# imedslab/OAProgressionMMF

Measured on AMD Instinct MI355X. Metric: knees/sec full XR+MRI+clin fusion train step, higher is better.
Workload: dtype f32; 1 GPU; syn3: XR1MR3C1CnnTrf train step (fwd+FocalLoss+bwd+Adam), per-GPU batch 8, global batch 8, BASELINE config 4 on BASELINE's synthetic tensors: XR 1x310x310 + 3 x MRI 1x160x384x384 (slice-major) + 9 clinical; random-init weights; parallelism=dp1, activation_recompute=012,012,01

## Files before the change

oaprogressionmmf_amd/csrc/koaf_conv.hip:

```cpp
#include "koaf_common.h"

namespace {

inline int64_t rup32(int64_t v) { return (v + 31) / 32 * 32; }

inline void set_fimg(KoafGemm* g, const KoafWImg* w, int R, int64_t K) {
    g->fmt = 1;
    g->A.fscale = KOAF_ACT_SCALE;
    g->B.amax = w->amax;
    if (!w->f) return;
    g->B.kind = 2; g->B.gather = 0;
    g->B.planes = w->f; g->B.ld = rup32(K); g->B.plane_stride = (int64_t)R * g->B.ld;
}

inline void set_aplanes(KoafOperand* a, const uint16_t* planes, int64_t plane_elems) {
    a->kind = 2; a->planes = planes; a->plane_stride = plane_elems; a->zeros = planes + 2 * plane_elems;
    a->ptr = nullptr; a->ptr2 = nullptr; a->tf = 0; a->sc = a->sh = a->sc2 = nullptr;
}

inline void set_gather(KoafOperand* o, int gather, int H, int W, int C, int CS, int PH, int PW, int KH, int KW, int stride, int pad_h,
                       int pad_w) {
    o->gather = gather;
    o->H = H; o->W = W; o->C = C; o->CS = CS;
    o->PH = PH; o->PW = PW;
    o->KH = KH; o->KW = KW; o->stride = stride; o->pad = pad_h; o->pad_w = pad_w;
}

inline bool is_pointwise(int KH, int KW, int stride, int pad) { return KH == 1 && KW == 1 && stride == 1 && pad == 0; }

struct WgradPlan { int bm, bn, splitk; };
inline WgradPlan wgrad_plan(int M, int N, int64_t K, int ctap, int batch) {
    WgradPlan p;
    p.bn = (N >= 128 && (ctap % 4) == 0) ? 128 : 64;
    p.bm = (M >= 128) ? 128 : 64;
    int64_t tiles = cdiv64(M, p.bm) * cdiv64(N, p.bn) * batch;
    int64_t sk = 1024 / tiles;
    int64_t kmax = cdiv64(K, 512);
    if (sk > kmax) sk = kmax;
    if (sk < 1) sk = 1;
    if (sk > 4096) sk = 4096;
    if (sk > 8) {
        int64_t best = sk & ~7ll;
        double beff = 0.0;
        for (int64_t c = ((sk * 3 / 4) + 7) & ~7ll; c <= 2 * sk && c <= kmax && c <= 4096; c += 8) {
            const int64_t blocks = tiles * c;
            const double eff = (double)blocks / (double)(cdiv64(blocks, 512) * 512);
            if (eff > beff + 0.02) { beff = eff; best = c; }
        }
        sk = best;
    }
    p.splitk = (int)sk;
    return p;
}

__global__ void __launch_bounds__(256) slab_reduce_b_kernel(const float* __restrict__ slabs, int ns, int64_t n,
                                                            float* __restrict__ out) {
    const int64_t i = ((int64_t)blockIdx.x * 256 + threadIdx.x) * 4;
    if (i >= n) return;
    const float* sb = slabs + (int64_t)blockIdx.y * ns * n;
    v4f a = *(const v4f*)(sb + i);
    for (int s = 1; s < ns; ++s) a += *(const v4f*)(sb + (int64_t)s * n + i);
    *(v4f*)(out + (int64_t)blockIdx.y * n + i) = a;
}

__global__ void __launch_bounds__(256) gconv_expand_kernel(const float* __restrict__ w, float* __restrict__ wexp,
                                                           int C, int Cg, float* __restrict__ amax) {
    const int64_t total = (int64_t)C * 9 * 64;
    unsigned mb = 0u;
    for (int64_t i = (int64_t)blockIdx.x * 256 + threadIdx.x; i < total; i += (int64_t)gridDim.x * 256) {
        const int ci = (int)(i & 63);
        int64_t r = i >> 6;
        const int tap = (int)(r % 9);
        const int co = (int)(r / 9);
        const int col = co & 63;
        const int g0 = (col / Cg) * Cg;
        float v = 0.f;
        if (ci >= g0 && ci < g0 + Cg) v = w[((int64_t)co * 9 + tap) * Cg + (ci - g0)];
        wexp[i] = v;
        mb = max(mb, koaf_absbits(v));
    }
    if (amax != nullptr) block_amax_raise_bits(mb, amax);
}
__global__ void __launch_bounds__(256) gconv_compress_kernel(const float* __restrict__ dwexp, float* __restrict__ dw,
                                                             int C, int Cg) {
    const int64_t total = (int64_t)C * 9 * Cg;
    for (int64_t i = (int64_t)blockIdx.x * 256 + threadIdx.x; i < total; i += (int64_t)gridDim.x * 256) {
        const int cg = (int)(i % Cg);
        int64_t r = i / Cg;
        const int tap = (int)(r % 9);
        const int co = (int)(r / 9);
        const int g0 = ((co & 63) / Cg) * Cg;
        dw[i] = dwexp[((int64_t)co * 9 + tap) * 64 + g0 + cg];
    }
}

}

int koaf_fwd_s2(const KoafGemm& g, void* stream);
static inline bool fwd_s2_ok(const KoafGemm& g, int KH, int KW, int stride, int pad, bool x_planes, bool tail, bool emit) {
    const KoafOperand& A = g.A;
    if (stride != 2 || KH != KW || !((KH == 1 && pad == 0) || (KH == 3 && pad == 1))) return false;
    if (g.fmt != 1 || g.B.kind != 2 || !g.B.planes || !g.B.amax || g.act16 != 0 || x_planes || tail || emit) return false;
    if (A.kind != 0 || A.gather != 1 || A.amax || (A.C % 32) != 0 || A.CS != A.C || (g.N % 128) != 0 || (g.M % 256) != 0 || g.K < 32) return false;
    if (A.tf != 0 && (A.tf != 1 || A.C > 1024 || !aligned16(A.sc) || !aligned16(A.sh))) return false;
    if (!aligned16(A.ptr) || !aligned16(g.B.planes) || !aligned16(g.C)) return false;
    return (int64_t)(g.M / (A.PH * A.PW)) * A.H * A.W < (1ll << 31);
}

extern "C" int koaf_conv2d_fwd(const float* x, const float* w, float* y, int32_t N, int32_t H, int32_t W, int32_t Cin,
                               int32_t Cout, int32_t KH, int32_t KW, int32_t stride, int32_t pad, const float* in_sc,
                               const float* in_sh, float* stats, int32_t* stats_rows, const float* stats_shift,
                               const KoafWImg* wimg, const uint16_t* x_planes, const KoafTail* tail, const KoafEmit* emit,
                               int32_t act16, void* stream) {
    KOAF_REQUIRE((x || x_planes) && w && y && N > 0 && Cin % 32 == 0 && Cout % 4 == 0, "koaf_conv2d_fwd: bad args (Cin=%d Cout=%d)",
                 Cin, Cout);
    KOAF_REQUIRE(!tail || (tail->idt && x && in_sc && in_sh && !x_planes && is_pointwise(KH, KW, stride, pad) && wimg &&
                           wimg->amax && wimg->f && (tail->idt_sc == nullptr) == (tail->idt_sh == nullptr)),
                 "koaf_conv2d_fwd: the fused bottleneck tail serves 1x1 / stride-1 convolutions with weight plane images, from x / in_sc / in_sh");
    KOAF_REQUIRE((in_sc == nullptr) == (in_sh == nullptr), "koaf_conv2d_fwd: in_sc/in_sh come together");
    const int OH = conv_out(H, KH, stride, pad), OW = conv_out(W, KW, stride, pad);
    const int64_t M = (int64_t)N * OH * OW;
    KOAF_REQUIRE(M < (1ll << 31), "koaf_conv2d_fwd: too many output pixels");
    KoafGemm g;
    zero_gemm(&g);
    g.A.ptr = x;
    g.A.kind = 0;
    if (is_pointwise(KH, KW, stride, pad) && !x_planes) {
        g.A.gather = 0;
        g.A.ld = Cin;
    } else
        set_gather(&g.A, 1, H, W, Cin, Cin, OH, OW, KH, KW, stride, pad, pad);
    if (in_sc) { g.A.tf = 1; g.A.sc = in_sc; g.A.sh = in_sh; }
    if (tail) { g.A.tf = 3; g.A.ptr2 = tail->idt; g.A.side = tail->y_out; g.A.sc2 = tail->idt_sc; g.A.sh2 = tail->idt_sc ? tail->idt_sh : nullptr; }
    g.B.ptr = w;
    g.B.kind = 0;
    g.B.ld = (int64_t)KH * KW * Cin;
    g.M = (int)M; g.N = Cout; g.K = KH * KW * Cin;
    if (wimg && wimg->amax) set_fimg(&g, wimg, Cout, g.K);
    if (x_planes) {
        KOAF_REQUIRE(g.A.gather == 1 && g.B.kind == 2, "koaf_conv2d_fwd: x_planes serve the gathered kernels and need wimg->f");
        set_aplanes(&g.A, x_planes, (int64_t)N * H * W * Cin);
    }
    g.C = y; g.ldc = Cout;
    g.stats = stats;
    g.stats_shift = stats ? stats_shift : nullptr;
    g.act16 = act16 ? 1 : 0;
    if (emit) {
        KOAF_REQUIRE(emit->planes && emit->sc && emit->sh && (Cout % 8) == 0, "koaf_conv2d_fwd: emit needs planes / sc / sh and Cout %% 8 == 0");
        g.out_planes = emit->planes; g.out_sc = emit->sc; g.out_sh = emit->sh; g.out_ps = M * Cout;
    }
    if (fwd_s2_ok(g, KH, KW, stride, pad, x_planes != nullptr, tail != nullptr, emit != nullptr)) {
        if (stats_rows) *stats_rows = g.M / 128;
        return koaf_fwd_s2(g, stream);
    }
    if (stats_rows) *stats_rows = koaf_gemm_part_rows(&g);
    return koaf_gemm(&g, stream);
}

extern "C" int32_t koaf_conv2d_stats_rows(int64_t M, int32_t Cout) { return (int32_t)cdiv64(M, 64); }

static void set_apply(KoafOperand* a, const KoafBnApply* ap, int C) {
    a->ptr = ap->dz; a->ptr2 = ap->c; a->tf = 2;
    a->sc = ap->coef; a->sc2 = ap->coef + 2 * (int64_t)C; a->sh = ap->coef + 3 * (int64_t)C;
    a->amax = ap->amax;
}

static void set_bnb(KoafGemm* g, const KoafBnb* b, float* part) {
    if (!b) return;
    g->bnb_amax = b->dz_amax;
    g->bnb_mode = b->mode;
    g->bnb_c = b->c; g->bnb_y = b->y; g->bnb_sc = b->sc; g->bnb_sh = b->sh;
    g->bnb_mean = b->mean; g->bnb_invstd = b->invstd;
    g->bnb2_c = b->c2; g->bnb2_mean = b->mean2; g->bnb2_invstd = b->invstd2;
    g->bnb_part = part;
}

extern "C" int32_t koaf_conv2d_dgrad_bnb_rows(int32_t N, int32_t H, int32_t W, int32_t Cin, int32_t stride) {
    if (stride == 2) {
        int64_t r = 0;
        for (int py = 0; py < 2; ++py)
            for (int px = 0; px < 2; ++px) r += cdiv64((int64_t)N * ((H - py + 1) / 2) * ((W - px + 1) / 2), 64);
        return (int32_t)r;
    }
    return (int32_t)cdiv64((int64_t)N * H * W, 64);
}

int koaf_dgrad_s2(const KoafGemm& g, void* stream);
static inline bool dgrad_s2_ok(const KoafGemm& g, int KH, int KW, int pad, int H, int W, const KoafBnb* bnb, bool dy_planes) {
    const KoafOperand& A = g.A;
    const bool f11 = KH == 1 && KW == 1 && pad == 0, f33 = KH == 3 && KW == 3 && pad == 1;
    if (!(f11 || f33) || (H & 1) || (W & 1) || (g.M % 256) != 0 || g.K < 32) return false;
    if (g.fmt != 1 || g.B.kind != 2 || !g.B.planes || !g.B.amax || !A.amax || g.act16 != 0 || g.residual) return false;
    if ((A.C % 32) != 0 || (g.N % 128) != 0 || !aligned16(g.C) || !aligned16(g.B.planes)) return false;
    if (bnb && (bnb->mode != 2 || bnb->c2 || !aligned16(bnb->c) || !aligned16(bnb->sc) || !aligned16(bnb->sh) || !aligned16(bnb->mean) ||
                !aligned16(bnb->invstd) || !aligned16(g.bnb_part)))
        return false;
    if (f33) return dy_planes && A.kind == 2 && aligned16(A.planes) && aligned16(A.zeros) && !(A.plane_stride & 7);
    if (dy_planes || bnb || A.kind != 0 || !aligned16(A.ptr)) return false;
    return A.tf == 0 || (A.tf == 2 && aligned16(A.ptr2) && aligned16(A.sc) && aligned16(A.sh) && aligned16(A.sc2));
}

extern "C" int koaf_conv2d_dgrad_bnb(const float* dy, const float* w, float* dx, int32_t N, int32_t H, int32_t W,
                                     int32_t Cin, int32_t Cout, int32_t KH, int32_t KW, int32_t stride, int32_t pad,
                                     const float* residual, const KoafBnb* bnb, float* part, int32_t* part_rows,
                                     const KoafWImg* wimg, const float* dy_amax, const KoafBnApply* dy_apply,
                                     const uint16_t* dy_planes, int32_t act16, void* stream) {
    KOAF_REQUIRE(!dy_planes || (wimg && wimg->amax && wimg->d && (dy_amax || dy_apply) && KH * KW > 1),
                 "koaf_conv2d_dgrad: dy_planes need the weight's D plane image, dy_amax and a gathered (KH*KW > 1) kernel");
    KOAF_REQUIRE((dy || dy_apply || dy_planes) && w && dx && N > 0 && Cout % 32 == 0 && Cin % 4 == 0, "koaf_conv2d_dgrad: bad args");
    KOAF_REQUIRE(!dy_apply || (dy_apply->dz && dy_apply->c && dy_apply->coef && dy_apply->amax && wimg && wimg->amax && wimg->d),
                 "koaf_conv2d_dgrad: dy_apply needs dz / c / coef / amax and the weight's D plane image");
    if (dy_apply) { dy = dy_apply->dz; dy_amax = dy_apply->amax; }
    if (bnb && bnb->dz_amax && hipMemsetAsync(bnb->dz_amax, 0, sizeof(float), (hipStream_t)stream) != hipSuccess) {
        koaf_set_error("koaf_conv2d_dgrad_bnb: memset failed");
        return KOAF_ELAUNCH;
    }
    const bool f16 = wimg && wimg->amax && dy_amax;
    const bool ps = f16 && wimg->d != nullptr;
    const uint16_t* w_dimg = ps ? wimg->d : nullptr;
    const int64_t dld = (int64_t)KH * KW * Cout, dps = (int64_t)Cin * dld;
    KOAF_REQUIRE(!bnb || (part && part_rows), "koaf_conv2d_dgrad_bnb: part / part_rows required");
    const int nsum = (bnb && bnb->c2) ? 3 : 2;
    int rows_done = 0;
    const int OH = conv_out(H, KH, stride, pad), OW = conv_out(W, KW, stride, pad);
    const int64_t M = (int64_t)N * H * W;
    KOAF_REQUIRE(M < (1ll << 31), "koaf_conv2d_dgrad: too many pixels");
    KoafGemm g;
    if (stride == 2) {
        bool all_done = false;
        for (int py = 0; py < 2 && !all_done; ++py)
            for (int px = 0; px < 2 && !all_done; ++px) {
                const int Hc = (H - py + 1) / 2, Wc = (W - px + 1) / 2;
                if (Hc <= 0 || Wc <= 0) continue;
                const int khs = (py + pad) & 1, kws = (px + pad) & 1;
                const int nkh = khs < KH ? (KH - khs + 1) / 2 : 0, nkw = kws < KW ? (KW - kws + 1) / 2 : 0;
                const int offy = (py + pad - khs) / 2, offx = (px + pad - kws) / 2;
                zero_gemm(&g);
                g.prec = 1;
                if (f16) { g.fmt = 1; g.A.amax = dy_amax; g.B.amax = wimg->amax; }
                g.A.ptr = dy; g.A.kind = 0;
                if (dy_apply) set_apply(&g.A, dy_apply, Cout);
                set_gather(&g.A, 2, OH, OW, Cout, Cout, Hc, Wc, nkh > 0 ? nkh : 1, nkw > 0 ? nkw : 1, 1, offy, offx);
                g.B.ptr = w + ((int64_t)khs * KW + kws) * Cin; g.B.kind = 1; g.B.gather = 3;
                g.B.C = Cout; g.B.ld = (int64_t)KH * KW * Cin;
                g.B.KW = g.A.KW; g.B.tap_stride = 2ll * Cin; g.B.tap_stride_h = 2ll * KW * Cin;
                if (ps) {
                    g.B.kind = 2; g.B.gather = 0;
                    g.B.planes = w_dimg + ((int64_t)khs * KW + kws) * Cout; g.B.ld = dld; g.B.plane_stride = dps;
                    g.B.tap_stride = 2ll * Cout; g.B.tap_stride_h = 2ll * KW * Cout;
                }
                if (dy_planes && nkh > 0 && nkw > 0) set_aplanes(&g.A, dy_planes, (int64_t)N * OH * OW * Cout);
                g.M = N * Hc * Wc; g.N = Cin; g.K = nkh * nkw * Cout;
                g.C = dx; g.ldc = Cin;
                g.residual = residual; g.ldr = Cin;
                g.cmap = 1; g.cm_PH = Hc; g.cm_PW = Wc; g.cm_H = H; g.cm_W = W; g.cm_py = py; g.cm_px = px;
                g.act16 = act16 ? 2 : 0;
                if (bnb) set_bnb(&g, bnb, part + (int64_t)rows_done * nsum * Cin);
                if (dgrad_s2_ok(g, KH, KW, pad, H, W, bnb, dy_planes != nullptr)) {
                    if (bnb) rows_done += g.M / 128;
                    int rc = koaf_dgrad_s2(g, stream);
                    if (rc != KOAF_OK) return rc;
                    all_done = KH == 1;
                    continue;
                }
                if (bnb) rows_done += koaf_gemm_part_rows(&g);
                int rc = koaf_gemm(&g, stream);
                if (rc != KOAF_OK) return rc;
            }
        if (part_rows) *part_rows = rows_done;
        return KOAF_OK;
    }
    zero_gemm(&g);
    g.prec = 1;
    if (f16) { g.fmt = 1; g.A.amax = dy_amax; g.B.amax = wimg->amax; }
    g.A.ptr = dy;
    g.A.kind = 0;
    if (dy_apply) set_apply(&g.A, dy_apply, Cout);
    g.B.ptr = w;
    g.B.kind = 1;
    if (is_pointwise(KH, KW, stride, pad)) {
        g.A.gather = 0;
        g.A.ld = Cout;
        g.B.gather = 0;
        g.B.ld = Cin;
    } else {
        set_gather(&g.A, 2, OH, OW, Cout, Cout, H, W, KH, KW, stride, pad, pad);
        g.B.gather = 3;
        g.B.C = Cout;
        g.B.ld = (int64_t)KH * KW * Cin;
        g.B.KW = KW;
        g.B.tap_stride = Cin;
        g.B.tap_stride_h = (int64_t)KW * Cin;
    }
    if (ps) {
        g.B.kind = 2; g.B.gather = 0; g.B.C = 0; g.B.tap_stride = g.B.tap_stride_h = 0;
        g.B.planes = w_dimg; g.B.ld = dld; g.B.plane_stride = dps;
    }
    if (dy_planes) set_aplanes(&g.A, dy_planes, (int64_t)N * OH * OW * Cout);
    g.M = (int)M; g.N = Cin; g.K = KH * KW * Cout;
    g.C = dx; g.ldc = Cin;
    g.residual = residual; g.ldr = Cin;
    if (bnb) {
        set_bnb(&g, bnb, part);
        *part_rows = koaf_gemm_part_rows(&g);
    }
    g.act16 = act16 ? 2 : 0;
// ... 204 lines not shown
```

oaprogressionmmf_amd/csrc/koaf_gemm.hip:

```cpp
#include "koaf_gemm_launch.h"
#include <stdlib.h>
#include <string.h>
#include <atomic>
#include <mutex>
#include <vector>

namespace {

__global__ void __launch_bounds__(256) slab_reduce_epi_kernel(const float* __restrict__ slabs, int nslab, int M, int N,
                                                              const float* __restrict__ bias,
                                                              const float* __restrict__ residual, int64_t ldr,
                                                              float* __restrict__ out, int64_t ldo) {
    const int N4 = N / 4;
    const int64_t total = (int64_t)M * N4;
    const int64_t n = (int64_t)M * N;
    for (int64_t i = (int64_t)blockIdx.x * 256 + threadIdx.x; i < total; i += (int64_t)gridDim.x * 256) {
        const int m = (int)(i / N4), c = (int)(i - (int64_t)m * N4) * 4;
        v4f a = *(const v4f*)(slabs + (int64_t)m * N + c);
        for (int s = 1; s < nslab; ++s) a += *(const v4f*)(slabs + (int64_t)s * n + (int64_t)m * N + c);
        if (bias) a += *(const v4f*)(bias + c);
        if (residual) a += *(const v4f*)(residual + (int64_t)m * ldr + c);
        *(v4f*)(out + (int64_t)m * ldo + c) = a;
    }
}

__global__ void __launch_bounds__(256) slab_reduce_kernel(const float* __restrict__ slabs, int nslab,
                                                          int64_t n, float* __restrict__ out) {
    __shared__ v4f red[4][64];
    const int cx = threadIdx.x & 63, gy = threadIdx.x >> 6;
    const int64_t i = ((int64_t)blockIdx.x * 64 + cx) * 4;
    const int s_per = (nslab + gridDim.y - 1) / gridDim.y;
    const int s0 = blockIdx.y * s_per, s1 = min(nslab, s0 + s_per);
    v4f a = {0.f, 0.f, 0.f, 0.f};
    if (i < n)
        for (int s = s0 + gy; s < s1; s += 4) a += *(const v4f*)(slabs + (int64_t)s * n + i);
    red[gy][cx] = a;
    __syncthreads();
    if (gy == 0 && i < n) {
        a = red[0][cx] + red[1][cx] + red[2][cx] + red[3][cx];
        if (gridDim.y == 1) *(v4f*)(out + i) = a;
        else *(v4f*)(out + (int64_t)blockIdx.y * n + i) = a;
    }
}

bool operand_vec_ok(const KoafOperand& o, int R, int K) {
    if (o.kind == 3) {
        return aligned16(o.planes) && aligned16(o.zeros) && o.zeros && !(o.plane_stride & 7) && !(o.bs0 & 7) && !(o.bs1 & 7) &&
               !(R & 7) && (o.gather ? (o.C > 0 && !(o.C & 7) && !(o.CS & 7) && o.KW > 0) : !(o.ld & 7));
    }
    if (o.kind == 2 && o.gather) {
        return aligned16(o.planes) && aligned16(o.zeros) && o.zeros && !(o.plane_stride & 7) && !(o.bs0 & 7) && !(o.bs1 & 7) &&
               o.C > 0 && !(o.C & 31) && !(o.CS & 7) && o.KW > 0 && (K % BK) == 0;
    }
    if (o.kind == 2) {
        if (!aligned16(o.planes) || (o.ld & 7) || (o.plane_stride & 7) || (o.bs0 & 7) || (o.bs1 & 7)) return false;
        if ((o.tap_stride & 7) || (o.tap_stride_h & 7) || o.C <= 0 || (o.C & 31) || o.KW <= 0) return false;
        return true;
    }
    if (!aligned16(o.ptr)) return false;
    if ((o.ld & 3) || (o.bs0 & 3) || (o.bs1 & 3)) return false;
    if (o.kind == 0) {
        if (K & 3) return false;
        if (o.gather && ((o.C & 31) || (o.CS & 3))) return false;
    } else {
        if (R & 3) return false;
        if (o.gather == 3 && ((o.C & 31) || (o.tap_stride & 3) || (o.tap_stride_h & 3))) return false;
        if (o.gather == 1 && ((o.C & 3) || (o.CS & 3))) return false;
    }
    if (o.tf && (!aligned16(o.sc) || !aligned16(o.sh))) return false;
    if (o.tf == 2 && (!aligned16(o.sc2) || !aligned16(o.ptr2))) return false;
    return true;
}

}

namespace {
std::atomic<int> g_log_on{0};
std::mutex g_log_mutex;
std::vector<KoafLaunchRec> g_log;
int64_t g_log_seen = 0;
constexpr size_t LOG_CAP = 4096;

}

void koaf_log_launch(const char* variant, const KoafGemm& g, dim3 grid, dim3 launched) {
    if (!g_log_on.load(std::memory_order_relaxed)) return;
    KoafLaunchRec r;
    memset(&r, 0, sizeof(r));
    strncpy(r.variant, variant, sizeof(r.variant) - 1);
    r.bm = g.bm; r.bn = g.bn;
    r.tiles = (int32_t)grid.x; r.grid_x = (int32_t)launched.x;
    r.splitk = (int32_t)launched.y; r.nbatch = (int32_t)launched.z;
    r.fmt = g.fmt; r.a_tf = g.A.tf; r.b_tf = g.B.tf; r.act16 = g.act16;
    r.M = g.M - g.m_base; r.N = g.N; r.K = g.K;
    r.emit = g.out_planes != nullptr;
    std::lock_guard<std::mutex> lock(g_log_mutex);
    ++g_log_seen;
    if (g_log.size() < LOG_CAP) g_log.push_back(r);
}

namespace {
int g_stream_mode = 1;
bool stream_ok(const KoafGemm& g) {
    return g_stream_mode == 1 && g.A.kind == 0 && g.A.gather == 0 && g.K >= 2 * BK && (g.K % (2 * BK)) == 0 && g.splitk == 1 &&
           g.nb0 * g.nb1 == 1 && (g.A.tf != 1 || g.K <= STREAM_TAB_K);
}
}

extern "C" int koaf_gemm_pick_tile(const KoafGemm* g, int32_t* bm, int32_t* bn) {
    int b_m = g->bm, b_n = g->bn;
    const int64_t batch = (int64_t)g->nb0 * g->nb1 * (g->splitk > 0 ? g->splitk : 1);
    if (b_n == 0) {
        b_n = (g->N >= 128) ? 128 : 64;
        if (g->B.kind == 1 && g->B.gather == 1 && (g->B.C % 64) != 0) b_n = 64;
    }
    if (b_m == 0) b_m = (g->M >= 128) ? 128 : 64;
    if (g->bm == 0 || g->bn == 0) {
        auto tiles = [&](int m, int n) { return cdiv64(g->M, m) * cdiv64(g->N, n) * batch; };
        constexpr int64_t fill = 384;
        if (g->bm == 0 && tiles(b_m, b_n) < fill && b_m == 128) b_m = 64;
        if (g->bn == 0 && tiles(b_m, b_n) < fill && b_n == 128) b_n = 64;
    }
    *bm = b_m;
    *bn = b_n;
    return KOAF_OK;
}

namespace {
int g_halo_mode = 1;

bool halo_ok(const KoafGemm& g) {
    const KoafOperand& a = g.A;
    return g_halo_mode != 0 && a.kind == 2 && (a.gather == 1 || a.gather == 2) && a.KH == 3 && a.KW == 3 && a.stride == 1 && a.pad == 1 &&
           a.pad_w == 1 && a.PH == a.H && a.PW == a.W && a.W <= halo_max_w(g.N >= 128 ? 128 : 64, 256) && a.H * a.W > 0 && (g.M % (a.H * a.W)) == 0 &&
           g.nb0 * g.nb1 == 1 && g.m_base == 0 && g.K == 9 * a.C && g.B.kind == 2 && g.fmt == 1 && !g.cmap && g.splitk == 1;
}

bool gemm_vec_ok(const KoafGemm& g) {
    bool vec = operand_vec_ok(g.A, g.M, g.K) && operand_vec_ok(g.B, g.N, g.K);
    if ((g.N & 3) || !aligned16(g.C) || (g.ldc & 3) || (g.cbs0 & 3) || (g.cbs1 & 3)) vec = false;
    if (g.residual && (!aligned16(g.residual) || (g.ldr & 3) || (g.rbs0 & 3) || (g.rbs1 & 3))) vec = false;
    if (g.bias && !aligned16(g.bias)) vec = false;
    return vec;
}

TilePlan plan_tiles(const KoafGemm& g) {
    TilePlan t;
    KoafGemm q = g;
    koaf_gemm_pick_tile(&q, &t.bm, &t.bn);
    t.vec = gemm_vec_ok(g);
    if (!t.vec) { t.bm = 64; t.bn = 64; }
    t.halo = t.vec && halo_ok(g);
    t.t2d = t.halo && g_halo_mode == 1 && g.A.C == 64 && (g.N == 64 || g.N == 128) && (g.A.W % 16) == 0 && (g.A.H % 8) == 0 &&
            g.A.zeros != nullptr;
    if (t.t2d) {
        t.halo = false;
        t.bm = 128;
        t.bn = 64;
    } else if (t.halo) {
        t.bn = g.N >= 128 ? 128 : 64;
        const bool fits128 = g.A.W <= halo_max_w(t.bn, 128);
        t.bm = (g_halo_mode == 3 || (g_halo_mode == 1 && g.A.C <= 64)) && fits128 ? 128 : 256;
    }
    t.part_rows = (int)cdiv64(g.M - g.m_base, t.bm);
    t.stream = t.vec && g.fmt == 1 && g.act16 == 0 && t.bm == 128 && operand_mode(g.A) == M_KC && operand_mode(g.B) == M_PS && !g.B.tf &&
               !(g.out_planes && g.A.tf == 2) && stream_ok(g);
    return t;
}
}

static void fill_defaults(KoafGemm& g) {
    if (g.nb0 < 1) g.nb0 = 1;
    if (g.nb1 < 1) g.nb1 = 1;
    if (g.splitk < 1) g.splitk = 1;
    if (g.A.CS == 0) g.A.CS = g.A.C;
    if (g.B.CS == 0) g.B.CS = g.B.C;
    if (g.stats_ld == 0) g.stats_ld = g.N;
    if (g.B.kind == 2 && g.B.C == 0) { g.B.C = ((g.K + BK - 1) / BK) * BK; g.B.KW = 1; }
}

namespace {
int launch_wplanes(const KoafGemm& g, const TilePlan& tp, dim3 grid, hipStream_t s) {
    switch (g.act16) {
        case 0: return koaf_launch_wplanes_act0(g, tp, grid, s);
        case 1: return koaf_launch_wplanes_act1(g, tp, grid, s);
        case 2: return koaf_launch_wplanes_act2(g, tp, grid, s);
    }
    return KOAF_NO_KERNEL;
}

int launch_planned(const KoafGemm& g, const TilePlan& tp, dim3 grid, hipStream_t s) {
    const int am = operand_mode(g.A), bm = operand_mode(g.B);
    if (g.out_planes && (tp.t2d || tp.halo)) { koaf_set_error("koaf_gemm: out_planes is not built for the 3x3 plane-image kernels"); return KOAF_EINVAL; }
    if ((tp.t2d || tp.halo) && g.act16 == 3) {
        koaf_set_error(tp.t2d ? "koaf_gemm: 2-D tile kernel with act16 = 3" : "koaf_gemm: halo kernel with act16 = 3");
        return KOAF_EINVAL;
    }
    if (tp.t2d || tp.halo) return launch_wplanes(g, tp, grid, s);
    if (g.fmt == 1) KOAF_REQUIRE(tp.vec, "koaf_gemm: the fp16 scheme needs the vector path (16-B aligned operands, K %% 4 == 0, N %% 4 == 0)");
    else if (!tp.vec && g.act16 != 0) { koaf_set_error("koaf_gemm: bf16 activation storage needs the vector path"); return KOAF_EINVAL; }
    int rc = KOAF_NO_KERNEL;
    if (tp.stream) rc = koaf_launch_stream(g, tp, grid, s);
    else if (g.out_planes) {
        if (g.fmt == 1 && am == M_KC && bm == M_PS) rc = launch_wplanes(g, tp, grid, s);
        if (rc == KOAF_NO_KERNEL) {
            koaf_set_error("koaf_gemm: out_planes is built for dense K-contiguous A x weight plane images on the fp16 scheme (1x1 forward convolutions); "
                           "got operand modes (%d,%d) tf=%d fmt=%d act16=%d", am, bm, g.A.tf, (int)(g.fmt == 1), g.act16);
            return KOAF_EINVAL;
        }
    }
    else if (bm == M_PS) rc = launch_wplanes(g, tp, grid, s);
    else if (am == M_PK) rc = koaf_launch_kmajor(g, tp, grid, s);
    else rc = g.fmt == 1 ? koaf_launch_fp16(g, tp, grid, s) : koaf_launch_bf16(g, tp, grid, s);
    if (rc == KOAF_NO_KERNEL) {
        koaf_set_error("koaf_gemm: operand mode pair (%d,%d) tf=(%d,%d) fmt=%d vec=%d act16=%d is not instantiated", am, bm, g.A.tf, g.B.tf,
                       (int)(g.fmt == 1), (int)tp.vec, g.act16);
        return KOAF_EINVAL;
    }
    return rc;
}
}

extern "C" int koaf_gemm_part_rows(const KoafGemm* gp) {
    KoafGemm g = *gp;
    fill_defaults(g);
    return plan_tiles(g).part_rows;
}

extern "C" int koaf_gemm(const KoafGemm* gp, void* stream) {
    KoafGemm g = *gp;
    KOAF_REQUIRE(g.M > 0 && g.N > 0 && g.K >= 0, "koaf_gemm: bad dims M=%d N=%d K=%d", g.M, g.N, g.K);
    KOAF_REQUIRE((g.A.kind >= 2 ? (const void*)g.A.planes : (const void*)g.A.ptr) &&
                 (g.B.kind >= 2 ? (const void*)g.B.planes : (const void*)g.B.ptr) && g.C, "koaf_gemm: null operand");
    fill_defaults(g);
    if (!g.status) g.status = koaf_status_ptr();
    KOAF_REQUIRE(!g.cmap || (g.splitk == 1 && !g.stats), "koaf_gemm: row map excludes split-K / stats");
    KOAF_REQUIRE(!g.bnb_mode || (g.splitk == 1 && !g.stats && g.nb0 * g.nb1 == 1 && g.bnb_c && g.bnb_mean &&
                                 g.bnb_invstd && g.bnb_part && (g.bnb_mode == 1 ? g.bnb_y != nullptr
                                                                                 : (g.bnb_sc && g.bnb_sh))),
                 "koaf_gemm: fused BN-backward epilogue needs c/mean/invstd/part (+y or sc/sh), no split-K/batch");
    KOAF_REQUIRE(g.splitk == 1 || (!g.bias && !g.residual && !g.stats),
                 "koaf_gemm: split-K writes raw slabs (no epilogue)");
    KOAF_REQUIRE((int64_t)g.nb0 * g.nb1 <= 65535 && g.splitk <= 65535, "koaf_gemm: batch/splitk too large");
    KOAF_REQUIRE(g.A.kind == 0 || (g.A.kind == 1 && g.A.gather == 0) || g.A.kind == 2 || (g.A.kind == 3 && g.A.gather == 0),
                 "koaf_gemm: A is K-contiguous fp32, K-major without gather, or activation plane images");
    KOAF_REQUIRE((g.A.kind == 3) == (g.B.kind == 3), "koaf_gemm: K-major plane images (kind 3) come as a pair");
    if (g.A.kind == 3)
        KOAF_REQUIRE(g.fmt == 1 && !g.A.tf && !g.B.tf && g.A.zeros && g.B.zeros && (g.B.gather == 0 || g.B.gather == 1),
                     "koaf_gemm: K-major plane images need fmt 1, no transform, the zero chunks; B.gather 0 | 1");
    if (g.A.kind == 2)
        KOAF_REQUIRE((g.A.gather == 1 || g.A.gather == 2) && g.B.kind == 2 && g.fmt == 1 && !g.A.tf && g.splitk == 1 && g.A.zeros,
                     "koaf_gemm: activation plane images (A.kind 2) need gather 1|2, a pre-split B, fmt 1, no transform, no split-K");
    KOAF_REQUIRE(!(g.A.kind == 0 && g.A.gather == 3) && !(g.B.kind == 0 && g.B.gather == 3),
                 "koaf_gemm: tapped gather needs a K-major operand");
    KOAF_REQUIRE(!(g.B.kind == 0 && g.B.gather), "koaf_gemm: K-contiguous B cannot be gathered");
    KOAF_REQUIRE(g.fmt == 0 || g.fmt == 1, "koaf_gemm: fmt must be 0 (bf16 x 3) or 1 (fp16 x 2)");
    KOAF_REQUIRE(g.A.tf >= 0 && g.A.tf <= 3 && g.B.tf >= 0 && g.B.tf <= 1, "koaf_gemm: tf is 0 | 1 (A, B) | 2 | 3 (A)");
    KOAF_REQUIRE(g.A.tf != 3 || (g.A.kind == 0 && g.A.gather == 0 && g.A.ptr2 && g.A.sc && g.A.sh && g.fmt == 1 && g.B.kind == 2 &&
                                 g.nb0 * g.nb1 == 1 && g.splitk == 1 && aligned16(g.A.ptr2) && (!g.A.side || aligned16(g.A.side)) &&
                                 (!g.A.sc2 || (g.A.sh2 && aligned16(g.A.sc2) && aligned16(g.A.sh2)))),
// ... 88 lines not shown
```

Baseline: 4.274 knees/s.

## Add dedicated persistent 1x1 conv forward kernel with fused BN-in and stats

Adds a specialized forward kernel for large pointwise (1x1, stride 1) convolutions. It uses 256-row tiles and a double-buffered LDS pipeline that converts f32 activations to split-f16 planes, with an optional persistent tile walk over 256 workgroups, and fuses the input BN transform and output statistics. The per-shape form comes from a small lookup table. The aim is to replace the generic GEMM path for the big MRI 1x1 convs, at the cost of more code and register/LDS pressure.

```diff
diff --git a/oaprogressionmmf_amd/csrc/koaf_conv.hip b/oaprogressionmmf_amd/csrc/koaf_conv.hip
--- a/oaprogressionmmf_amd/csrc/koaf_conv.hip
+++ b/oaprogressionmmf_amd/csrc/koaf_conv.hip
@@ -105,6 +105,20 @@
     if (A.tf != 0 && (A.tf != 1 || A.C > 1024 || !aligned16(A.sc) || !aligned16(A.sh))) return false;
     if (!aligned16(A.ptr) || !aligned16(g.B.planes) || !aligned16(g.C)) return false;
     return (int64_t)(g.M / (A.PH * A.PW)) * A.H * A.W < (1ll << 31);
+}
+
+int koaf_fwd1(const KoafGemm& g, int form, void* stream);
+int koaf_fwd1_form(int K, int N);
+bool koaf_stream_on();
+static inline int fwd1_ok(const KoafGemm& g, int KH, int KW, int stride, int pad, bool x_planes, bool tail, bool emit) {
+    const KoafOperand& A = g.A;
+    if (!is_pointwise(KH, KW, stride, pad) || !koaf_stream_on()) return -1;
+    if (g.fmt != 1 || g.B.kind != 2 || !g.B.planes || !g.B.amax || g.act16 != 0 || x_planes || tail || emit) return -1;
+    if (A.kind != 0 || A.gather != 0 || A.amax || A.ld != g.K || (g.K % 32) != 0 || g.K < 64 || (g.N % 128) != 0) return -1;
+    if ((g.M % 256) != 0 || g.M < 65536) return -1;
+    if (A.tf != 0 && (A.tf != 1 || g.K > 1024 || !aligned16(A.sc) || !aligned16(A.sh))) return -1;
+    if (!aligned16(A.ptr) || !aligned16(g.B.planes) || !aligned16(g.C)) return -1;
+    return koaf_fwd1_form(g.K, g.N);
 }
 
 extern "C" int koaf_conv2d_fwd(const float* x, const float* w, float* y, int32_t N, int32_t H, int32_t W, int32_t Cin,
@@ -152,6 +166,10 @@
     if (fwd_s2_ok(g, KH, KW, stride, pad, x_planes != nullptr, tail != nullptr, emit != nullptr)) {
         if (stats_rows) *stats_rows = g.M / 128;
         return koaf_fwd_s2(g, stream);
+    }
+    if (const int form = fwd1_ok(g, KH, KW, stride, pad, x_planes != nullptr, tail != nullptr, emit != nullptr); form >= 0) {
+        if (stats_rows) *stats_rows = g.M / 128;
+        return koaf_fwd1(g, form, stream);
     }
     if (stats_rows) *stats_rows = koaf_gemm_part_rows(&g);
     return koaf_gemm(&g, stream);
diff --git a/oaprogressionmmf_amd/csrc/koaf_fwd1.hip b/oaprogressionmmf_amd/csrc/koaf_fwd1.hip
--- /dev/null
+++ b/oaprogressionmmf_amd/csrc/koaf_fwd1.hip
@@ -0,0 +1,372 @@
+#include <hip/hip_runtime.h>
+#include <stdint.h>
+#include <type_traits>
+#include "koaf.h"
+#include "koaf_pieces.h"
+
+namespace {
+struct F1Params {
+    const float* x;
+    const float* sc;
+    const float* sh;
+    float a_scale;
+    const unsigned short* wf;
+    int64_t w_ps, w_ld;
+    const float* w_amax;
+    float alpha;
+    float* y;
+    float* stats;
+    const float* shift;
+    int64_t stats_ld;
+    uint32_t* status;
+    int M, N, K;
+    int tiles;
+    int part_row0;
+};
+
+constexpr int F1_NT = 512;
+constexpr int F1_BM = 256;
+constexpr int F1_TAB_C = 1024;
+constexpr int F1_CUS = 256;
+
+template <int BN, int TF, int WALK>
+__global__ void __launch_bounds__(F1_NT) fwd1_kernel(const F1Params p) {
+    constexpr int BM = F1_BM, WGN = 2;
+    constexpr int WM = BM / 4, WN = BN / WGN, TM = WM / 32, TN = WN / 32;
+    constexpr int A_PL = plane_dwords(BM, true), B_PL = BN * 16;
+    constexpr int A_ELEMS = 2 * A_PL, B_ELEMS = 2 * B_PL, STAGE = A_ELEMS + B_ELEMS;
+    constexpr int TAB = TF == 1 ? 2 * F1_TAB_C : 0;
+    constexpr int LDC_S = BN + 4;
+    static_assert((2 * STAGE + TAB) * 4 <= 160 * 1024, "two stages of both operands and the table in LDS");
+    static_assert(128 * LDC_S <= 2 * STAGE && 8 * BN <= 2 * STAGE, "staging half and statistics reduction reuse the stages");
+    __shared__ __attribute__((aligned(16))) unsigned smem[2 * STAGE + (TAB ? TAB : 4)];
+    [[maybe_unused]] const float* const tab = reinterpret_cast<const float*>(smem + 2 * STAGE);
+
+    const int ntn = p.N / BN;
+    int tile, tile_end;
+    {
+        const unsigned ntx = gridDim.x, v = blockIdx.x;
+        const unsigned q = ntx >> 3, rem = ntx & 7, x = v & 7, j = v >> 3;
+        const unsigned b = x * q + (x < rem ? x : rem) + j;
+        if constexpr (WALK) {
+            tile = (int)((uint64_t)b * (unsigned)p.tiles / ntx);
+            tile_end = (int)((uint64_t)(b + 1u) * (unsigned)p.tiles / ntx);
+        } else {
+            tile = (int)b;
+            tile_end = tile + 1;
+        }
+    }
+    const int K = p.K, nstep = K / BK;
+
+    const float sca = p.a_scale, scb = scale_of_amax(*p.w_amax);
+    float alpha = p.alpha / (sca * scb);
+    if (!koaf_bits_finite(koaf_absbits(*p.w_amax))) {
+        alpha = __uint_as_float(0x7fc00000u);
+        if (blockIdx.x == 0 && threadIdx.x == 0) koaf_status_add(p.status, 1, 1u);
+    }
+
+    const int t = threadIdx.x;
+    int lane, wm, wn;
+    unsigned kq, ar;
+    unsigned aoff;
+    unsigned boff, bdst;
+    auto thread_indices = [&]() {
+        int tk = t;
+        if constexpr (WALK) asm volatile("" : "+v"(tk));
+        lane = tk & 63;
+        wm = (tk >> 6) / WGN; wn = (tk >> 6) % WGN;
+        kq = (unsigned)tk & 7u; ar = (unsigned)tk >> 3;
+        aoff = ar * (unsigned)K + 4u * kq;
+        boff = ((unsigned)tk >> 2) * (unsigned)p.w_ld + 8u * ((unsigned)tk & 3u);
+        bdst = ((unsigned)tk >> 2) * 16u + 4u * (((unsigned)tk & 3u) ^ (((unsigned)tk >> 4) & 3u));
+    };
+    thread_indices();
+
+    constexpr int NUA = 4;
+    const unsigned arow = 64u * (unsigned)K;
+    v4f ra[NUA];
+    [[maybe_unused]] unsigned satmax = 0u;
+    v4f ca = {0.f, 0.f, 0.f, 0.f}, cb = ca;
+    const float* a_base;
+    const unsigned short* b_base;
+    int ki = 0;
+    auto tile_bases = [&](int tl, const float*& ab, const unsigned short*& bb) {
+        const int tn_ = tl % ntn, tm_ = tl / ntn;
+        ab = p.x + (int64_t)tm_ * BM * K;
+        bb = p.wf + (int64_t)tn_ * BN * p.w_ld;
+    };
+    auto issue_a = [&](int i) { ra[i] = *(const v4f*)(a_base + (ki + i * arow) + aoff); };
+    auto convert_a = [&](int i, unsigned* S, bool live) {
+        constexpr float HMAX = 65504.f;
+        v4f v;
+#pragma unroll
+        for (int j = 0; j < 4; ++j) {
+            float x = ra[i][j];
+            if constexpr (TF == 1) {
+                x = fmaf(x, ca[j], cb[j]);
+                x = __builtin_amdgcn_fmed3f(x, 0.f, HMAX);
+            } else {
+                x = __builtin_amdgcn_fmed3f(x * sca, -HMAX, HMAX);
+            }
+            v[j] = x;
+        }
+        unsigned pl[2][2];
+        split2h(v, pl);
+        if constexpr (TF == 1) {
+            typedef unsigned short u16x2 __attribute__((ext_vector_type(2)));
+#pragma unroll
+            for (int d = 0; d < 2; ++d)
+                satmax = __builtin_bit_cast(unsigned, __builtin_elementwise_max(__builtin_bit_cast(u16x2, satmax),
+                                                                                 __builtin_bit_cast(u16x2, live ? pl[0][d] : 0u)));
+        }
+        const unsigned off = (ar + 64u * i) * 20u + 2u * kq;
+#pragma unroll
+        for (int q = 0; q < 2; ++q) *(uint2*)&S[q * A_PL + off] = make_uint2(pl[q][0], pl[q][1]);
+    };
+    auto load_coef = [&](int coff) {
+        if constexpr (TF == 1) {
+            ca = *(const v4f*)&tab[coff + 4 * (int)kq];
+            cb = *(const v4f*)&tab[F1_TAB_C + coff + 4 * (int)kq];
+        }
+    };
+
+    constexpr int NUB = BN / 64;
+    v4i rb[NUB];
+    auto issue_b = [&](int u) { rb[u] = *(const v4i*)(b_base + ((u & 1) * p.w_ps + (int64_t)(128 * (u >> 1)) * p.w_ld + ki) + boff); };
+    auto store_b = [&](int u, unsigned* S) { *(v4i*)&S[A_ELEMS + (u & 1) * B_PL + (u >> 1) * (128 * 16) + bdst] = rb[u]; };
+
+    v16f acc[TM][TN];
+
+    constexpr int NUT = NUA + NUB, NG = 2 * TN;
+    int ccoff = 0;
+    [[maybe_unused]] const float* a_next = nullptr;
+    [[maybe_unused]] const unsigned short* b_next = nullptr;
+    auto unit = [&](int u, unsigned* S, bool live) {
+        if (u < NUA) { convert_a(u, S, live); issue_a(u); }
+        else { store_b(u - NUA, S); issue_b(u - NUA); }
+    };
+    auto lgkm0_barrier = [&]() {
+        __builtin_amdgcn_s_waitcnt(0xC07F);
+        asm volatile("s_barrier" ::: "memory");
+    };
+    auto advance = [&]() {
+        ki += BK;
+        if (ki >= K) {
+            ki = 0;
+            if constexpr (WALK) { a_base = a_next; b_base = b_next; }
+        }
+        ccoff += BK;
+        if (ccoff >= K) ccoff = 0;
+    };
+    auto step = [&](int cur, bool live, auto units_c) {
+        constexpr bool UNITS = decltype(units_c)::value;
+        const unsigned* Au = smem + cur * STAGE;
+        const unsigned* Bu = Au + A_ELEMS;
+        unsigned* Sn = smem + (cur ^ 1) * STAGE;
+        if constexpr (UNITS) load_coef(ccoff);
+#pragma unroll
+        for (int g = 0; g < 2; ++g) {
+            v4i ap[TM][2];
+#pragma unroll
+            for (int i = 0; i < TM; ++i)
+#pragma unroll
+                for (int q = 0; q < 2; ++q) ap[i][q] = frag_load<BM, true>(Au + q * A_PL, wm * WM + 32 * i, g, lane);
+#pragma unroll
+            for (int jn = 0; jn < TN; ++jn) {
+                v4i bp[2];
+#pragma unroll
+                for (int q = 0; q < 2; ++q) bp[q] = frag_load_ps(Bu + q * B_PL, wn * WN + 32 * jn, g, lane);
+                constexpr int PAH[3] = {1, 0, 0}, PBH[3] = {0, 1, 0};
+#pragma unroll
+                for (int term = 0; term < 3; ++term)
+#pragma unroll
+                    for (int i = 0; i < TM; ++i)
+                        acc[i][jn] = __builtin_amdgcn_mfma_f32_32x32x16_f16(__builtin_bit_cast(h16x8, ap[i][PAH[term]]),
+                                                                            __builtin_bit_cast(h16x8, bp[PBH[term]]), acc[i][jn], 0, 0, 0);
+                if constexpr (UNITS) {
+                    const int grp = g * TN + jn;
+#pragma unroll
+                    for (int u = 0; u < NUT; ++u)
+                        if (u * NG / NUT == grp) unit(u, Sn, live);
+                    __builtin_amdgcn_sched_barrier(0x104);
+                }
+            }
+        }
+        if constexpr (UNITS) advance();
+        lgkm0_barrier();
+    };
+
+    if constexpr (TF == 1) {
+        float* tw = reinterpret_cast<float*>(smem + 2 * STAGE);
+        for (int c = t; c < K; c += F1_NT) { tw[c] = p.sc[c] * sca; tw[F1_TAB_C + c] = p.sh[c] * sca; }
+    }
+    tile_bases(tile, a_base, b_base);
+#pragma unroll
+    for (int i = 0; i < NUA; ++i) issue_a(i);
+#pragma unroll
+    for (int u = 0; u < NUB; ++u) issue_b(u);
+    if constexpr (TF == 1) __syncthreads();
+
+    const bool do_stats = p.stats != nullptr;
+    float* Cs = reinterpret_cast<float*>(smem);
+    constexpr int C4 = BN / 4, RPP = F1_NT / C4;
+
+#pragma unroll 1
+    for (; tile < tile_end; ++tile) {
+        const int tn = tile % ntn, tm = tile / ntn;
+        const int m0 = tm * BM, n0 = tn * BN;
+        if constexpr (WALK) {
+            tile_bases(tile + 1 < tile_end ? tile + 1 : tile, a_next, b_next);
+            thread_indices();
+        }
+        ki = BK;
+        ccoff = 0;
+        load_coef(0);
+#pragma unroll
+        for (int u = 0; u < NUT; ++u) unit(u, smem, true);
+        advance();
+#pragma unroll
+        for (int i = 0; i < TM; ++i)
+#pragma unroll
+            for (int j = 0; j < TN; ++j)
+#pragma unroll
+                for (int e = 0; e < 16; ++e) acc[i][j][e] = 0.f;
+        lgkm0_barrier();
+        if constexpr (WALK) {
+#pragma unroll 1
+            for (int s = 0; s + 1 < nstep; ++s) step(s & 1, true, std::true_type{});
+            step((nstep - 1) & 1, false, std::false_type{});
+        } else {
+#pragma unroll 1
+            for (int s = 0; s < nstep; ++s) step(s & 1, s + 1 < nstep, std::true_type{});
+        }
+
+        if constexpr (TF == 1) {
+            if (((satmax & 0xffffu) >= 0x7bffu) | ((satmax >> 16) >= 0x7bffu)) koaf_status_add(p.status, 0, 1u);
+            satmax = 0u;
+        }
+
+        int te = t;
+        if constexpr (WALK) asm volatile("" : "+v"(te));
+        const int wm = (te >> 6) / WGN, wn = (te >> 6) % WGN, r = te & 31, h = (te >> 5) & 1;
+        const int c4 = te % C4, rr = te / C4;
+        float s1[TM][TN], s2[TM][TN], kshift[TN];
+#pragma unroll
+        for (int jn = 0; jn < TN; ++jn) {
+#pragma unroll
+            for (int i = 0; i < TM; ++i) s1[i][jn] = s2[i][jn] = 0.f;
+            kshift[jn] = (do_stats && p.shift) ? p.shift[n0 + wn * WN + 32 * jn + r] : 0.f;
+        }
+        v4f bv = {0.f, 0.f, 0.f, 0.f};
+        asm volatile("" : "+v"(bv));
+#pragma unroll
+        for (int hh = 0; hh < 2; ++hh) {
+            if ((wm >> 1) == hh) {
+#pragma unroll
+                for (int i = 0; i < TM; ++i)
+#pragma unroll
+                    for (int jn = 0; jn < TN; ++jn)
+#pragma unroll
+                        for (int e = 0; e < 16; ++e) {
+                            const float v = alpha * acc[i][jn][e];
+                            s1[i][jn] += v - kshift[jn];
+                            s2[i][jn] = fmaf(v - kshift[jn], v - kshift[jn], s2[i][jn]);
+                            Cs[((wm & 1) * WM + 32 * i + (e & 3) + 8 * (e >> 2) + 4 * h) * LDC_S + wn * WN + 32 * jn + r] = v;
+                        }
+            }
+            __syncthreads();
+            float* const Yp = p.y + (int64_t)(m0 + 128 * hh) * p.N + n0 + 4 * c4;
+#pragma unroll 4
+            for (int row = rr; row < 128; row += RPP) {
+                const v4f v = *(const v4f*)&Cs[row * LDC_S + 4 * c4] + bv;
+                __builtin_nontemporal_store(v, (v4f*)(Yp + (int64_t)row * p.N));
+            }
+            __syncthreads();
+        }
+        if (do_stats) {
+            float* red = Cs;
+#pragma unroll
+            for (int jn = 0; jn < TN; ++jn) {
+                float a1 = s1[0][jn] + __shfl_xor(s1[0][jn], 32, 64);
+                float a2 = s2[0][jn] + __shfl_xor(s2[0][jn], 32, 64);
+#pragma unroll
+                for (int i = 1; i < TM; ++i) {
+                    a1 += s1[i][jn] + __shfl_xor(s1[i][jn], 32, 64);
+                    a2 += s2[i][jn] + __shfl_xor(s2[i][jn], 32, 64);
+                }
+                if (h == 0) {
+                    red[(wm * 2 + 0) * BN + wn * WN + 32 * jn + r] = a1;
+                    red[(wm * 2 + 1) * BN + wn * WN + 32 * jn + r] = a2;
+                }
+            }
+            __syncthreads();
+            if (te < 2 * BN) {
+                const int hh = te / BN, c = te % BN;
+                float a1 = red[(4 * hh + 0) * BN + c], a2 = red[(4 * hh + 1) * BN + c];
+                a1 += red[(4 * hh + 2) * BN + c];
+                a2 += red[(4 * hh + 3) * BN + c];
+                float* st = p.stats + (int64_t)(p.part_row0 + 2 * tm + hh) * 2 * p.stats_ld;
+                st[n0 + c] = a1;
+                st[p.stats_ld + n0 + c] = a2;
+            }
+            if constexpr (WALK) __syncthreads();
+        }
+    }
+}
+
+template <int BN, int WALK>
+int f1_launch(const F1Params& p, int tf, dim3 grid, hipStream_t s) {
+    if (tf) hipLaunchKernelGGL((fwd1_kernel<BN, 1, WALK>), grid, dim3(F1_NT), 0, s, p);
+    else hipLaunchKernelGGL((fwd1_kernel<BN, 0, WALK>), grid, dim3(F1_NT), 0, s, p);
+    return koaf_check_launch("koaf_fwd1");
+}
+}
+
+void koaf_log_launch(const char* variant, const KoafGemm& g, dim3 grid, dim3 launched);
+
+int koaf_fwd1_form(int K, int N) {
+#ifdef KOAF_FWD1_FORCE
+    return KOAF_FWD1_FORCE;
+#else
+    struct Row { int K, N, form; };
+    static const Row rows[] = {
+        {64, 256, -1},
+        {128, 512, 1}, {256, 1024, 1}, {512, 2048, 0}, {256, 128, 1}, {512, 256, 1},
+    };
+    for (const Row& r : rows)
+        if (r.K == K && r.N == N) return r.form;
+    return 1;
+#endif
+}
+
+int koaf_fwd1(const KoafGemm& g, int form, void* stream) {
+    const KoafOperand& A = g.A;
+    const KoafOperand& B = g.B;
+    KOAF_REQUIRE(g.fmt == 1 && g.act16 == 0 && A.kind == 0 && A.gather == 0 && A.ptr && !A.ptr2 && !A.amax &&
+                 (A.tf == 0 || (A.tf == 1 && A.sc && A.sh && g.K <= F1_TAB_C)) && A.ld == g.K &&
+                 B.kind == 2 && B.gather == 0 && B.planes && B.amax && !B.tf && g.C && g.ldc == g.N && g.splitk <= 1 && g.nb0 * g.nb1 <= 1 &&
+                 !g.bias && !g.residual && !g.cmap && !g.bnb_mode && !g.out_planes && g.m_base == 0 && g.stats_bs == 0 &&
+                 g.M % F1_BM == 0 && g.N % 128 == 0 && g.K >= 2 * BK && g.K % BK == 0 && g.K <= 8192 && B.ld == g.K && (form == 0 || form == 1),
+                 "koaf_fwd1: bad args");
+    F1Params p;
+    p.x = A.ptr; p.sc = A.sc; p.sh = A.sh;
+    p.a_scale = A.fscale != 0.f ? A.fscale : 1.f;
+    p.wf = B.planes; p.w_ps = B.plane_stride; p.w_ld = B.ld; p.w_amax = B.amax;
+    p.alpha = g.alpha;
+    p.y = g.C;
+    p.stats = g.stats; p.shift = g.stats ? g.stats_shift : nullptr; p.stats_ld = g.stats_ld ? g.stats_ld : g.N;
+    p.status = g.status ? g.status : koaf_status_ptr();
+    p.M = g.M; p.N = g.N; p.K = g.K;
+    p.part_row0 = g.part_row0;
+    const int bn = (g.N % 256) == 0 ? 256 : 128;
+    const int64_t tiles = (int64_t)(g.M / F1_BM) * (g.N / bn);
+    KOAF_REQUIRE(tiles < (1ll << 31), "koaf_fwd1: too many tiles");
+    p.tiles = (int)tiles;
+    const dim3 grid((unsigned)tiles), launched(form ? (unsigned)(tiles < F1_CUS ? tiles : F1_CUS) : (unsigned)tiles);
+    KoafGemm rec = g;
+    rec.bm = F1_BM; rec.bn = bn;
+    koaf_log_launch("koaf_fwd1", rec, grid, launched);
+    hipStream_t s = (hipStream_t)stream;
+    if (form) return bn == 256 ? f1_launch<256, 1>(p, A.tf, launched, s) : f1_launch<128, 1>(p, A.tf, launched, s);
+    return bn == 256 ? f1_launch<256, 0>(p, A.tf, launched, s) : f1_launch<128, 0>(p, A.tf, launched, s);
+}
diff --git a/oaprogressionmmf_amd/csrc/koaf_gemm.hip b/oaprogressionmmf_amd/csrc/koaf_gemm.hip
--- a/oaprogressionmmf_amd/csrc/koaf_gemm.hip
+++ b/oaprogressionmmf_amd/csrc/koaf_gemm.hip
@@ -106,6 +106,8 @@
            g.nb0 * g.nb1 == 1 && (g.A.tf != 1 || g.K <= STREAM_TAB_K);
 }
 }
+
+bool koaf_stream_on() { return g_stream_mode == 1; }
 
 extern "C" int koaf_gemm_pick_tile(const KoafGemm* g, int32_t* bm, int32_t* bn) {
     int b_m = g->bm, b_n = g->bn;
```

New measurement: 4.333 knees/s (median of 6 runs). +1.4%, better.
